# midas-journal/midas-journal-740

Measured on NVIDIA B200. Metric: Gvoxels/s, higher is better.
Workload: dtype f32

## Files before the change

### midas-journal-740_b200/csrc/cuberille_capi.cu

```cuda
#include <cuda_runtime.h>

#include <algorithm>
#include <cmath>
#include <cstdarg>
#include <cstdio>
#include <cstdlib>
#include <cstring>
#include <limits>
#include <new>
#include <string>
#include <type_traits>
#include <vector>

#include "../../include/cuberille_c.h"
#include "cbr_common.cuh"
#include "k_classify.cuh"
#include "k_segscan.cuh"
#include "k_generate.cuh"
#include "k_faces.cuh"
#include "k_project.cuh"
#include "k_sweep.cuh"
#include "k_fused.cuh"
#include "k_vertices.cuh"

// ... 827 lines not shown
  }
  const uint64_t tot_v = h->h_info[kInfoTotV], tot_f = h->h_info[kInfoTotF];
  if (tot_v >= (1ull << 32) || tot_f >= (1ull << 32))
    return fail(h, CUB_ERR_OVERFLOW, "more than 2^32 vertices or faces in one handle (%llu, %llu): split into z-slabs",
                (unsigned long long)tot_v, (unsigned long long)tot_f);
  h->n_active = h->h_info[kInfoTotC];
  h->ghost_f = h->h_info[kInfoMarkF];
  h->ghost_v = h->h_info[kInfoGhostV];
  h->n_points = h->h_info[kInfoPoints];
  h->n_quads = h->h_info[kInfoQuads];
  h->point_base = h->h_info[kInfoPointBase];
  h->cell_base = h->h_info[kInfoCellBase];
  h->flags = h->h_info[kInfoFlags];
  h->warning.clear();
  if (h->flags & kFlagEmptyInteriorSlice)
    h->warning = "an empty voxel slice lies between occupied slices: the reference filter merges vertices of different corner "
                 "planes there (its lookup-plane rotation only advances on inside voxels, txx:155-161); this mesh follows the "
                 "intended rule and may differ from the reference's";
  h->counted = true;
  return CUB_OK;
}

const int kNeedSizes = -1000;

int emit_mode(cub_handle h) {
  const cub_params& P = h->params;
  if (!P.generate_triangles) return kEmitQuads;
  return (P.project_vertices || h->geom.oriented) ? kEmitScratchQuads : kEmitTrisFixed;
}

int size_vertex_buffers(cub_handle h) {
  const size_t n_pts_all = (size_t)(h->ghost_v + h->n_points);
  CUB_TRY(ensure(h, h->points, 3 * (n_pts_all + n_pts_all / 16)));
  if (!h->raster) {
    CUB_TRY(ensure(h, h->perm, (size_t)h->n_active + (size_t)h->n_active / 16));
    CUB_TRY(ensure(h, h->vtx, h->points.cap / 3));
  }
  return CUB_OK;
}

int emit_vertex_stage(cub_handle h, bool exact) {
  const Grid& g = h->g;
  const int mode = emit_mode(h);
  const int nz = h->zs1 - h->owner_z_min;
  if (exact) {
    CUB_TRY(size_vertex_buffers(h));
    if (h->n_quads == 0) { h->vertices_done = true; return CUB_OK; }
  } else if (!h->points.p || (!h->raster && (!h->perm.p || !h->vtx.p))) {
    return kNeedSizes;
  }
  h->vertices_done = true;
  h->projected = false;
  if (!h->caps_checked) {
    CU_TRY(h, launch_step(h, k_check_caps, dim3(1), dim3(32), true, h->d_info, make_caps(h, ~0ull)));
  }
  const bool ghost_points = (mode == kEmitScratchQuads) && h->owner_z_min < h->zs0;
  if (!h->raster) {
    const size_t cap = std::min(h->points.cap / 3, h->vtx.cap);
    const size_t n_ids = exact ? (size_t)(h->ghost_v + h->n_points) : cap;
    const unsigned n_blocks = (unsigned)((n_ids + kVertexBlockIds - 1) / kVertexBlockIds);
    CUB_TRY(ensure(h, h->vsl, (size_t)nz + 1 + (cap + kVertexBlockIds - 1) / kVertexBlockIds + 1));
    {
      AssignArgs a{};
      a.cnt = h->cnt.p; a.own = h->own.p; a.seg = h->seg.p; a.cofs = h->cofs.p;
      a.Wx = g.Wx; a.EY = h->EY; a.EW = h->EW; a.NS = h->NS; a.z_begin = h->owner_z_min;
      a.ghost_row_end = (unsigned)((size_t)h->zs0 * h->EY);
      a.vtx = h->vtx.p; a.info = h->d_info;
      const int rows = kAssignThreads / 32;
      const dim3 grid((g.Wx + 31) / 32, (h->EY + rows - 1) / rows, nz + 1);
      CU_TRY(h, launch_step(h, k_assign, grid, dim3(kAssignThreads), true, a));
    }
    if (n_blocks > 0) {
      SliceIndexArgs si{};
      si.seg = h->seg.p; si.plane_segs = (size_t)h->EY * h->NS; si.z_first = h->owner_z_min; si.nz = nz;
      si.slice_first = h->vsl.p; si.block_slice = h->vsl.p + nz + 1; si.n_blocks = n_blocks; si.ids_per_block = kVertexBlockIds;
      const unsigned si_threads = n_blocks > (unsigned)nz + 1 ? n_blocks : (unsigned)nz + 1;
      CU_TRY(h, launch_step(h, k_slice_index, dim3((si_threads + 255) / 256), dim3(256), true, si));
      VertexArgs a{};
      a.vtx = h->vtx.p; a.caps = make_caps(h, ~0ull); a.write_ghost_points = ghost_points ? 1 : 0;
      a.info = h->d_info;
      a.slice_first = si.slice_first; a.block_slice = si.block_slice; a.z_first = h->owner_z_min;
      a.act = h->act.p; a.cofs = h->cofs.p; a.EY = h->EY; a.EW = h->EW;
      a.plane_lo = h->zs0; a.plane_hi = h->zs1; a.geom = h->geom;
      a.coff[0] = (int)(h->i0[0] - h->pad); a.coff[1] = (int)(h->i0[1] - h->pad); a.coff[2] = (int)(h->i0[2] + g.zg0 - h->pad);
      a.points = h->points.p; a.perm = h->perm.p;
      CU_TRY(h, launch_step(h, h->geom.oriented ? k_vertices<true> : k_vertices<false>, dim3(n_blocks), dim3(256), true, a));
    }
  } else {
    RasterPointArgs a{};
    a.act = h->act.p; a.cofs = h->cofs.p; a.seg = h->seg.p; a.EY = h->EY; a.EW = h->EW; a.NS = h->NS; a.Wc = (g.X + 32) / 32;
    a.plane_lo = h->zs0; a.plane_hi = h->zs1;
    a.point_plane_lo = (ghost_points || h->own_z0 == 0) ? h->zs0 : h->zs0 + 1;
    a.coff[0] = (int)(h->i0[0] - h->pad); a.coff[1] = (int)(h->i0[1] - h->pad); a.coff[2] = (int)(h->i0[2] + g.zg0 - h->pad);
    a.geom = h->geom; a.points = h->points.p; a.info = h->d_info;
    const dim3 grid((unsigned)h->NS, (h->EY + 7) / 8, a.plane_hi - a.plane_lo + 1);
    auto kern = h->geom.oriented ? k_points_raster<true> : k_points_raster<false>;
    kern<<<grid, 256, 0, h->stream>>>(a);
    h->launches++;
    CU_TRY(h, cudaGetLastError());
  }
  return CUB_OK;
}

int emit_launch(cub_handle h, int id_bytes, bool exact) {
  CU_TRY(h, cudaSetDevice(h->device));
  const cub_params& P = h->params;
  const Grid& g = h->g;
  const bool tri = P.generate_triangles != 0, proj = P.project_vertices != 0, cd = P.save_pixel_as_cell_data != 0;
  const int mode = emit_mode(h);
  h->verts_per_cell = tri ? 3 : 4;
  h->id_bytes = id_bytes;
  const size_t quad_bytes = (size_t)(tri ? 6 : 4) * id_bytes;
  const size_t cd_bytes = (size_t)(tri ? 2 : 1) * h->pix_bytes;
  if (exact) {
    h->n_cells = tri ? 2 * h->n_quads : h->n_quads;
    if (id_bytes == 4 && h->point_base + h->n_points > (1ull << 32))
      return fail(h, CUB_ERR_OVERFLOW, "point ids up to %llu do not fit 32 bits", (unsigned long long)(h->point_base + h->n_points));
    const size_t nq = (size_t)h->n_quads + (size_t)h->n_quads / 16;
    CUB_TRY(ensure(h, h->cells, nq * quad_bytes));
    if (mode == kEmitScratchQuads) CUB_TRY(ensure(h, h->quads, nq));
    if (cd) CUB_TRY(ensure(h, h->celldata, nq * cd_bytes));
  } else if (!h->cells.p || (mode == kEmitScratchQuads && !h->quads.p) || (cd && !h->celldata.p)) {
    return kNeedSizes;
  }
  size_t quads_cap = h->cells.cap / quad_bytes;
  if (mode == kEmitScratchQuads) quads_cap = std::min(quads_cap, h->quads.cap);
  if (cd) quads_cap = std::min(quads_cap, h->celldata.cap / cd_bytes);
  if (proj && h->projected) h->vertices_done = false;
  if (exact && !h->vertices_done) CUB_TRY(size_vertex_buffers(h));

  if (h->timing) cudaEventRecord(h->ev[4], h->stream);
  CU_TRY(h, launch_step(h, k_check_caps, dim3(1), dim3(32), true, h->d_info, make_caps(h, quads_cap)));
  h->caps_checked = true;
  const bool ghost_points = (mode == kEmitScratchQuads) && h->owner_z_min < h->zs0;
  if (!exact || h->n_quads > 0) {
    Timer t(h, 2);
    if (!h->vertices_done) {
      const int rc = emit_vertex_stage(h, exact);
      if (rc != CUB_OK) return rc;
    }
    {
      if (h->wait_before_faces) CU_TRY(h, cudaStreamWaitEvent(h->stream, h->wait_before_faces, 0));
      FaceArgs a{};
      a.bits = h->bits.p; a.g = g; a.EY = h->EY; a.EW = h->EW; a.NS = h->NS;
      a.z_begin = h->zs0; a.z_end = h->zs1;
      a.act = h->act.p; a.cofs = h->cofs.p; a.seg = h->seg.p; a.perm = h->raster ? nullptr : h->perm.p;
      a.info = h->d_info;
      a.cells = (mode == kEmitScratchQuads) ? (void*)h->quads.p : (void*)h->cells.p;
      a.mode = mode;
      a.vol = cd ? h->d_vol : nullptr;
      a.vX = h->gv.X; a.vY = h->gv.Y; a.vpad = h->pad; a.vzpad = h->zpad_lo;
      a.celldata = cd ? h->celldata.p : nullptr;
      a.pix_bytes = h->pix_bytes;
      const dim3 blocks((g.Wx + 31) / 32, (g.Y + kFaceThreads / 32 - 1) / (kFaceThreads / 32), h->zs1 - h->zs0);
      const bool pdl = h->wait_before_faces == nullptr;
      void (*kern)(FaceArgs);
      if (mode == kEmitScratchQuads) kern = cd ? k_faces<uint32_t, kEmitScratchQuads, true> : k_faces<uint32_t, kEmitScratchQuads, false>;
      else if (mode == kEmitQuads && id_bytes == 4) kern = cd ? k_faces<uint32_t, kEmitQuads, true> : k_faces<uint32_t, kEmitQuads, false>;
      else if (mode == kEmitQuads) kern = cd ? k_faces<unsigned long long, kEmitQuads, true> : k_faces<unsigned long long, kEmitQuads, false>;
      else if (id_bytes == 4) kern = cd ? k_faces<uint32_t, kEmitTrisFixed, true> : k_faces<uint32_t, kEmitTrisFixed, false>;
      else kern = cd ? k_faces<unsigned long long, kEmitTrisFixed, true> : k_faces<unsigned long long, kEmitTrisFixed, false>;
      CU_TRY(h, launch_step(h, kern, blocks, dim3(kFaceThreads), pdl, a));
    }
    t.stop();
  }
  if (proj && (!exact || h->n_points > 0)) {
    Timer t(h, 3);
    CUB_TRY(launch_project(h, h->points.p, h->points.cap / 3, true, ghost_points));
    h->projected = true;
    t.stop();
  }
  if (mode == kEmitScratchQuads && (!exact || h->n_quads > 0)) {
    Timer t(h, 4);
    const size_t want = exact ? (size_t)h->n_quads : quads_cap;
    const unsigned blocks = (unsigned)std::max<size_t>(1, std::min<size_t>((want + 255) / 256, (size_t)h->num_sms * 16));
    if (id_bytes == 4)
      k_split_quads<uint32_t><<<blocks, 256, 0, h->stream>>>(h->quads.p, h->points.p, (uint32_t*)h->cells.p, h->d_info);
    else
      k_split_quads<unsigned long long><<<blocks, 256, 0, h->stream>>>(h->quads.p, h->points.p, (unsigned long long*)h->cells.p, h->d_info);
    h->launches++;
    CU_TRY(h, cudaGetLastError());
    t.stop();
  }
  if (h->timing) {
    cudaEventRecord(h->ev[5], h->stream);
    cudaEventSynchronize(h->ev[5]);
    cudaEventElapsedTime(&h->ms[6], h->ev[4], h->ev[5]);
  }
  h->emitted = true;
  h->emit_unverified = !exact;
  return CUB_OK;
}

int verify_emit(cub_handle h) {
  if (!h->counted) CUB_TRY(count_finish(h));
  if (h->emit_unverified) {
    h->emit_unverified = false;
    const cub_params& P = h->params;
    h->n_cells = P.generate_triangles ? 2 * h->n_quads : h->n_quads;
    if (h->flags & kFlagBufferOverflow) {
      h->vertices_done = false;
      CUB_TRY(emit_launch(h, h->id_bytes, true));
      CU_TRY(h, cudaStreamSynchronize(h->stream));
    } else if (h->id_bytes == 4 && h->point_base + h->n_points > (1ull << 32)) {
      return fail(h, CUB_ERR_OVERFLOW, "point ids up to %llu do not fit 32 bits", (unsigned long long)(h->point_base + h->n_points));
    }
  }
  return CUB_OK;
}

}

extern "C" {

int cub_count(cub_handle h, const cub_params* p, uint64_t* n_points, uint64_t* n_quads) {
  if (!h) return CUB_ERR_INVALID;
  CUB_TRY(count_launch(h, p));
  CUB_TRY(count_finish(h));
  if (n_points) *n_points = h->n_points;
  if (n_quads) *n_quads = h->n_quads;
  return CUB_OK;
}

int cub_count_async(cub_handle h, const cub_params* p) {
  if (!h) return CUB_ERR_INVALID;
  return count_launch(h, p);
}

int cub_projection_halo(const cub_params* p, const double spacing[3], uint64_t* below, uint64_t* above) {
  if (!p || !below || !above) return CUB_ERR_INVALID;
  double sp[3] = {1.0, 1.0, 1.0};
  if (spacing) for (int a = 0; a < 3; ++a) sp[a] = spacing[a];
  if (!p->project_vertices) { *below = 2; *above = 1; return CUB_OK; }
  double ms = sp[0];
  for (int a = 1; a < 3; ++a) ms = sp[a] > ms ? sp[a] : ms;
  const double step = p->step_length < 0.0 ? ms * 0.25 : p->step_length;
  projection_reach(*p, step, 1.0 / sp[2], below, above);
  return CUB_OK;
}

int cub_set_id_base(cub_handle h, uint64_t point_id_base, uint64_t cell_id_base) {
  if (!h) return CUB_ERR_INVALID;
  h->point_base = point_id_base;
  h->cell_base = cell_id_base;
  if (h->count_queued) {
    CU_TRY(h, cudaSetDevice(h->device));
    k_set_bases<<<1, 32, 0, h->stream>>>(h->d_info, point_id_base, cell_id_base);
    h->launches++;
    CU_TRY(h, cudaGetLastError());
  }
  return CUB_OK;
}

int cub_emit_vertices(cub_handle h) {
  if (!h) return CUB_ERR_INVALID;
  if (!h->count_queued) return fail(h, CUB_ERR_INVALID, "cub_emit_vertices before cub_count");
  CU_TRY(h, cudaSetDevice(h->device));
  if (h->vertices_done || h->timing) return CUB_OK;
  const int rc = emit_vertex_stage(h, h->counted);
  return rc == kNeedSizes ? CUB_OK : rc;
}

int cub_emit(cub_handle h, int id_bytes) {
  if (!h) return CUB_ERR_INVALID;
  if (!h->count_queued) return fail(h, CUB_ERR_INVALID, "cub_emit before cub_count");
  if (id_bytes != 4 && id_bytes != 8) return fail(h, CUB_ERR_INVALID, "id_bytes must be 4 or 8");
  if (!h->counted) CUB_TRY(count_finish(h));
  return emit_launch(h, id_bytes, true);
}

int cub_emit_async(cub_handle h, int id_bytes) {
  if (!h) return CUB_ERR_INVALID;
  if (!h->count_queued) return fail(h, CUB_ERR_INVALID, "cub_emit_async before cub_count_async");
  if (id_bytes != 4 && id_bytes != 8) return fail(h, CUB_ERR_INVALID, "id_bytes must be 4 or 8");
  if (!h->counted && !h->timing) {
    const int rc = emit_launch(h, id_bytes, false);
    if (rc != kNeedSizes) return rc;
  }
  if (!h->counted) CUB_TRY(count_finish(h));
  return emit_launch(h, id_bytes, true);
}

int cub_finish(cub_handle h, uint64_t* n_points, uint64_t* n_cells) {
  if (!h) return CUB_ERR_INVALID;
  if (!h->count_queued) return fail(h, CUB_ERR_INVALID, "cub_finish: nothing has been queued");
  CUB_TRY(verify_emit(h));
  if (!h->emit_unverified) CU_TRY(h, cudaStreamSynchronize(h->stream));
  if (n_points) *n_points = h->n_points;
  if (n_cells) *n_cells = h->params.generate_triangles ? 2 * h->n_quads : h->n_quads;
  return CUB_OK;
}

int cub_device_counts(cub_handle h, const uint64_t** counts) {
  if (!h || !counts) return CUB_ERR_INVALID;
  *counts = reinterpret_cast<const uint64_t*>(h->d_info + kInfoPoints);
  return CUB_OK;
}

const char* cub_last_warning(cub_handle h) { return h ? h->warning.c_str() : ""; }

int cub_run(cub_handle h, const cub_params* p, int id_bytes, uint64_t* n_points, uint64_t* n_cells) {
  uint64_t np = 0, nq = 0;
  CUB_TRY(cub_count(h, p, &np, &nq));
  CUB_TRY(cub_emit(h, id_bytes));
  if (n_points) *n_points = h->n_points;
  if (n_cells) *n_cells = h->n_cells;
  return CUB_OK;
// ... 201 lines not shown
```

### midas-journal-740_b200/csrc/k_faces.cuh

```cuda
#pragma once
#include "cbr_common.cuh"
#include "k_segscan.cuh"

namespace cbr {

enum { kEmitQuads = 0, kEmitTrisFixed = 1, kEmitScratchQuads = 2 };

struct FaceArgs {
  const uint32_t* bits;
  Grid g;
  int EY, EW, NS;
  int z_begin, z_end;
  const uint32_t* act;
  const uint32_t* cofs;
  const uint4* seg;
  const uint32_t* perm;
  unsigned long long* info;
  void* cells;
  int mode;
  const void* vol;
  int vX, vY, vpad, vzpad;
  void* celldata;
  int pix_bytes;
};

template <typename IdT>
__device__ __forceinline__ void store_tri_pair(IdT* c, IdT a0, IdT a1, IdT a2, IdT b0, IdT b1, IdT b2) {
  if (sizeof(IdT) == 4) {
    uint2* d = reinterpret_cast<uint2*>(c);
    d[0] = make_uint2((uint32_t)a0, (uint32_t)a1);
    d[1] = make_uint2((uint32_t)a2, (uint32_t)b0);
    d[2] = make_uint2((uint32_t)b1, (uint32_t)b2);
  } else {
    ulonglong2* d = reinterpret_cast<ulonglong2*>(c);
    d[0] = make_ulonglong2((unsigned long long)a0, (unsigned long long)a1);
    d[1] = make_ulonglong2((unsigned long long)a2, (unsigned long long)b0);
    d[2] = make_ulonglong2((unsigned long long)b1, (unsigned long long)b2);
  }
}

template <typename IdT, int MODE>
__device__ __forceinline__ void write_cell(const FaceArgs& a, uint32_t fidx, IdT v0, IdT v1, IdT v2, IdT v3) {
  if (MODE == kEmitScratchQuads) {
    reinterpret_cast<uint4*>(a.cells)[fidx] = make_uint4((uint32_t)v0, (uint32_t)v1, (uint32_t)v2, (uint32_t)v3);
    return;
  }
  IdT* c = reinterpret_cast<IdT*>(a.cells);
  if (MODE == kEmitQuads) {
    c += (size_t)fidx * 4;
    if (sizeof(IdT) == 4) {
      *reinterpret_cast<uint4*>(c) = make_uint4((uint32_t)v0, (uint32_t)v1, (uint32_t)v2, (uint32_t)v3);
    } else {
      reinterpret_cast<ulonglong2*>(c)[0] = make_ulonglong2((unsigned long long)v0, (unsigned long long)v1);
      reinterpret_cast<ulonglong2*>(c)[1] = make_ulonglong2((unsigned long long)v2, (unsigned long long)v3);
    }
  } else {
    c += (size_t)fidx * 6;
    store_tri_pair<IdT>(c, v0, v1, v3, v1, v2, v3);
  }
}

__device__ __forceinline__ unsigned long long load_pixel(const void* vol, size_t voxel, int pix_bytes) {
  switch (pix_bytes) {
    case 1: return __ldg(reinterpret_cast<const uint8_t*>(vol) + voxel);
    case 2: return __ldg(reinterpret_cast<const uint16_t*>(vol) + voxel);
    case 4: return __ldg(reinterpret_cast<const uint32_t*>(vol) + voxel);
    default: return __ldg(reinterpret_cast<const unsigned long long*>(vol) + voxel);
  }
}

template <int MODE>
__device__ __forceinline__ void write_celldata(const FaceArgs& a, uint32_t fidx, unsigned long long pix) {
  const bool two = (MODE != kEmitQuads);
  const size_t c = two ? 2 * (size_t)fidx : (size_t)fidx;
  switch (a.pix_bytes) {
    case 1: { uint8_t* d = reinterpret_cast<uint8_t*>(a.celldata) + c; d[0] = (uint8_t)pix; if (two) d[1] = (uint8_t)pix; break; }
    case 2: { uint16_t* d = reinterpret_cast<uint16_t*>(a.celldata) + c; d[0] = (uint16_t)pix; if (two) d[1] = (uint16_t)pix; break; }
    case 4: { uint32_t* d = reinterpret_cast<uint32_t*>(a.celldata) + c; d[0] = (uint32_t)pix; if (two) d[1] = (uint32_t)pix; break; }
    default: { unsigned long long* d = reinterpret_cast<unsigned long long*>(a.celldata) + c; d[0] = pix; if (two) d[1] = pix; break; }
  }
}

constexpr int kFaceThreads = 128;

struct FaceSmem {
  uint4 ctx[4][kFaceThreads / 32][32];
  uint16_t queue[kFaceThreads / 32][1024];
};

template <typename IdT, int MODE, bool CD>
__global__ void __launch_bounds__(kFaceThreads, 12) k_faces(const FaceArgs a) {
  pdl_enter();
  __shared__ FaceSmem sm;
  const bool fits = emission_fits(a.info);
  const Grid& g = a.g;
  const int lane = threadIdx.x & 31, warp = threadIdx.x >> 5;
  const int sgm = blockIdx.x, w = sgm * 32 + lane, y = blockIdx.y * (kFaceThreads / 32) + warp, zl = a.z_begin + blockIdx.z;

  uint32_t F[6] = {0, 0, 0, 0, 0, 0};
  const int plane = a.EY * a.EW;
  const uint32_t e00 = ((uint32_t)zl * (uint32_t)a.EY + (uint32_t)y) * (uint32_t)a.EW + (uint32_t)w;
  uint32_t A[4] = {0, 0, 0, 0}, C[4] = {0, 0, 0, 0};
  uint32_t fseg = 0;
  const unsigned long long id_delta = __ldg(a.info + kInfoIdDelta);
  const uint32_t ghost_f = (uint32_t)__ldg(a.info + kInfoMarkF);
  {
    const bool valid = w < g.Wx && y < g.Y;
    if (y < g.Y) fseg = __ldg(&a.seg[((uint32_t)zl * (uint32_t)a.EY + (uint32_t)y) * (uint32_t)a.NS + (uint32_t)sgm].y);
    const uint32_t* __restrict__ row = a.bits + (((uint32_t)zl * (uint32_t)g.Y + (uint32_t)y) * (uint32_t)g.Wp + (uint32_t)w);
    const int zgl = zl + g.zg0;
    const int sw = g.Y * g.Wp;
    const int dym = (y > 0) ? -g.Wp : 0, dyp = (y < g.Y - 1) ? g.Wp : 0;
    const int dzm = (zgl > 0 && zl > 0) ? -sw : 0, dzp = (zgl < g.Zg - 1 && zl < g.Zl - 1) ? sw : 0;
    uint32_t c0 = 0, nym = 0, nyp = 0, nzm = 0, nzp = 0, edge = 0;
    if (valid) {
#pragma unroll
      for (int k = 0; k < 4; ++k) {
        const uint32_t e = e00 + (uint32_t)((k >> 1) * plane + (k & 1) * a.EW);
        A[k] = __ldg(a.act + e);
        C[k] = __ldg(a.cofs + e);
      }
      c0 = __ldg(row);
      nym = __ldg(row + dym); nyp = __ldg(row + dyp); nzm = __ldg(row + dzm); nzp = __ldg(row + dzp);
      if (lane == 0 && w > 0) edge = __ldg(row - 1);
      if (lane == 31 && w < g.Wx - 1) edge = __ldg(row + 1);
    }
    const uint32_t up = __shfl_up_sync(0xffffffffu, c0, 1), dn = __shfl_down_sync(0xffffffffu, c0, 1);
    if (valid) {
      const uint32_t XB = g.X & 31;
      const uint32_t vc = (w == g.Wx - 1 && XB) ? ((1u << XB) - 1u) : ~0u;
      const uint32_t c = c0 & vc;
      const uint32_t prev = (w == 0) ? (c0 << 31) : (lane == 0 ? edge : up);
      const uint32_t next = (w == g.Wx - 1) ? (c0 >> 31) : (lane == 31 ? edge : dn);
      F[0] = c & ~__funnelshift_l(prev, c0, 1);
      F[1] = c & ~nym;
      F[2] = c & ~__funnelshift_r(c0, next, 1);
      F[3] = c & ~nyp;
      F[4] = c & ~nzm;
      F[5] = c & ~nzp;
    }
  }
  uint32_t U = F[0] | F[1] | F[2] | F[3] | F[4] | F[5];
  const uint32_t nvox = __popc(U);
  const uint32_t nf = __popc(F[0]) + __popc(F[1]) + __popc(F[2]) + __popc(F[3]) + __popc(F[4]) + __popc(F[5]);
  uint32_t s0 = nvox | (nf << 16);
  const uint32_t m0 = s0;
#pragma unroll
  for (int o = 1; o < 32; o <<= 1) {
    const uint32_t t0 = __shfl_up_sync(0xffffffffu, s0, o);
    if (lane >= o) s0 += t0;
  }
  const uint32_t total = __shfl_sync(0xffffffffu, s0, 31) & 0xffffu;
  if (!fits) return;
  if (total == 0) return;

  if (U) {
    s0 -= m0;
    sm.ctx[0][warp][lane] = make_uint4(A[0], A[1], A[2], A[3]);
    sm.ctx[1][warp][lane] = make_uint4(C[0], C[1], C[2], C[3]);
    sm.ctx[2][warp][lane] = make_uint4(F[0], F[1], F[2], F[3]);
    sm.ctx[3][warp][lane] = make_uint4(F[4], F[5], fseg + (s0 >> 16) - ghost_f, 0u);
    uint32_t pos = s0 & 0xffffu;
    uint16_t* q = sm.queue[warp];
    const uint32_t tag = (uint32_t)lane << 5;
    while (U) {
      const int b = __ffs(U) - 1;
      U &= U - 1;
      q[pos++] = (uint16_t)(tag | (uint32_t)b);
    }
  }
  __syncwarp();

  for (uint32_t s = lane; s < total; s += 32) {
    const uint32_t it = sm.queue[warp][s];
    const uint32_t src = it >> 5, b = it & 31u;
    const uint4 A4 = sm.ctx[0][warp][src], C4 = sm.ctx[1][warp][src], Fa = sm.ctx[2][warp][src], Fb = sm.ctx[3][warp][src];
    const uint32_t A[4] = {A4.x, A4.y, A4.z, A4.w}, C[4] = {C4.x, C4.y, C4.z, C4.w};
    const uint32_t Fm[6] = {Fa.x, Fa.y, Fa.z, Fa.w, Fb.x, Fb.y};
    const uint32_t bit = 1u << b, below = bit - 1u;
    uint32_t fi = Fb.z;
#pragma unroll
    for (int f = 0; f < 6; ++f) fi += __popc(Fm[f] & below);
    uint32_t vid[8];
#pragma unroll
    for (int k = 0; k < 4; ++k) {
      const int oz = k >> 1, oy = k & 1;
      const uint32_t s0 = C[k] + __popc(A[k] & below);
      const uint32_t s1 = s0 + ((A[k] >> b) & 1u);
      vid[oz * 4 + (oy ? 3 : 0)] = s0;
      vid[oz * 4 + (oy ? 2 : 1)] = s1;
    }
    const bool f0 = Fm[0] & bit, f1 = Fm[1] & bit, f2 = Fm[2] & bit, f3 = Fm[3] & bit, f4 = Fm[4] & bit, f5 = Fm[5] & bit;
    if (a.perm) {
      const bool need[8] = {f0 || f1 || f4, f1 || f2 || f4, f2 || f3 || f4, f0 || f3 || f4,
                            f0 || f1 || f5, f1 || f2 || f5, f2 || f3 || f5, f0 || f3 || f5};
#pragma unroll
      for (int l = 0; l < 8; ++l)
        if (need[l]) vid[l] = __ldg(a.perm + vid[l]);
    }
    const unsigned long long voxel =
        CD ? load_pixel(a.vol, ((size_t)(zl - a.vzpad) * a.vY + (size_t)(y - a.vpad)) * a.vX +
                                           (size_t)((sgm * 32 + src) * 32 + b - a.vpad), a.pix_bytes) : 0ull;
    IdT fid[8];
#pragma unroll
    for (int l = 0; l < 8; ++l) fid[l] = MODE == kEmitScratchQuads ? (IdT)vid[l] : (IdT)(vid[l] + id_delta);
    if (f0) { write_cell<IdT, MODE>(a, fi, fid[0], fid[4], fid[7], fid[3]); if (CD) write_celldata<MODE>(a, fi, voxel); ++fi; }
    if (f1) { write_cell<IdT, MODE>(a, fi, fid[0], fid[1], fid[5], fid[4]); if (CD) write_celldata<MODE>(a, fi, voxel); ++fi; }
    if (f2) { write_cell<IdT, MODE>(a, fi, fid[1], fid[2], fid[6], fid[5]); if (CD) write_celldata<MODE>(a, fi, voxel); ++fi; }
    if (f3) { write_cell<IdT, MODE>(a, fi, fid[2], fid[3], fid[7], fid[6]); if (CD) write_celldata<MODE>(a, fi, voxel); ++fi; }
    if (f4) { write_cell<IdT, MODE>(a, fi, fid[0], fid[3], fid[2], fid[1]); if (CD) write_celldata<MODE>(a, fi, voxel); ++fi; }
    if (f5) { write_cell<IdT, MODE>(a, fi, fid[4], fid[5], fid[6], fid[7]); if (CD) write_celldata<MODE>(a, fi, voxel); ++fi; }
  }
}

template <typename IdT>
__global__ void __launch_bounds__(256) k_split_quads(const uint4* __restrict__ quads, const float* __restrict__ points,
                                                     IdT* __restrict__ tris, unsigned long long* __restrict__ info) {
  if (!emission_fits(info)) return;
  const size_t n_quads = (size_t)__ldg(info + kInfoQuads);
  const unsigned long long id_delta = __ldg(info + kInfoIdDelta);
  for (size_t i = (size_t)blockIdx.x * blockDim.x + threadIdx.x; i < n_quads; i += (size_t)gridDim.x * blockDim.x) {
    const uint4 q = quads[i];
    const uint32_t id[4] = {q.x, q.y, q.z, q.w};
    float p[4][3];
#pragma unroll
    for (int k = 0; k < 4; ++k)
#pragma unroll
      for (int c = 0; c < 3; ++c) p[k][c] = __ldg(points + 3 * (size_t)id[k] + c);
    double d02 = 0.0, d13 = 0.0;
#pragma unroll
    for (int c = 0; c < 3; ++c) {
      const double a = __dadd_rn((double)p[0][c], -(double)p[2][c]);
      d02 = __dadd_rn(d02, __dmul_rn(a, a));
      const double b = __dadd_rn((double)p[1][c], -(double)p[3][c]);
      d13 = __dadd_rn(d13, __dmul_rn(b, b));
    }
    IdT v[4];
#pragma unroll
    for (int k = 0; k < 4; ++k) v[k] = (IdT)((unsigned long long)id[k] + id_delta);
    IdT* c = tris + i * 6;
    const bool first = d02 >= d13;
    store_tri_pair<IdT>(c, v[0], v[1], first ? v[3] : v[2], first ? v[1] : v[0], v[2], v[3]);
  }
}

}
```

Baseline: 540.8.

## Process four bit-words per lane in face kernel with chunked queue and batched emission

Each lane of the face-emission kernel now handles four consecutive 32-bit occupancy words, loaded with uint4 vector loads, so a warp covers four rows instead of one. The per-warp voxel queue becomes a 512-entry ring that is filled and drained in chunks. Emission gathers two queued voxels before writing, so the perm and pixel loads can overlap. The goal is fewer load instructions, more work per thread and better latency hiding, at the cost of higher register and shared-memory use, which is why occupancy is lowered from 12 to 5 blocks per SM.

```diff
diff --git a/midas-journal-740_b200/csrc/cuberille_capi.cu b/midas-journal-740_b200/csrc/cuberille_capi.cu
--- a/midas-journal-740_b200/csrc/cuberille_capi.cu
+++ b/midas-journal-740_b200/csrc/cuberille_capi.cu
@@ -1003,7 +1003,7 @@
       a.vX = h->gv.X; a.vY = h->gv.Y; a.vpad = h->pad; a.vzpad = h->zpad_lo;
       a.celldata = cd ? h->celldata.p : nullptr;
       a.pix_bytes = h->pix_bytes;
-      const dim3 blocks((g.Wx + 31) / 32, (g.Y + kFaceThreads / 32 - 1) / (kFaceThreads / 32), h->zs1 - h->zs0);
+      const dim3 blocks((g.Wx + 31) / 32, (g.Y + kFaceRows - 1) / kFaceRows, h->zs1 - h->zs0);
       const bool pdl = h->wait_before_faces == nullptr;
       void (*kern)(FaceArgs);
       if (mode == kEmitScratchQuads) kern = cd ? k_faces<uint32_t, kEmitScratchQuads, true> : k_faces<uint32_t, kEmitScratchQuads, false>;
diff --git a/midas-journal-740_b200/csrc/k_faces.cuh b/midas-journal-740_b200/csrc/k_faces.cuh
--- a/midas-journal-740_b200/csrc/k_faces.cuh
+++ b/midas-journal-740_b200/csrc/k_faces.cuh
@@ -82,67 +82,167 @@
 }
 
 constexpr int kFaceThreads = 128;
+constexpr int kFaceWordsPerLane = 4;
+constexpr int kFaceLanesPerSeg = 32 / kFaceWordsPerLane;
+constexpr int kFaceSegsPerWarp = 32 / kFaceLanesPerSeg;
+constexpr int kFaceRows = kFaceThreads / 32 * kFaceSegsPerWarp;
+constexpr int kFaceSlots = 32 * kFaceWordsPerLane;
+constexpr int kFaceQueue = 512;
+constexpr int kFaceEmitDepth = 2;
 
 struct FaceSmem {
-  uint4 ctx[4][kFaceThreads / 32][32];
-  uint16_t queue[kFaceThreads / 32][1024];
+  uint4 ctx[4][kFaceThreads / 32][kFaceSlots];
+  uint16_t queue[kFaceThreads / 32][kFaceQueue];
 };
 
+__device__ __forceinline__ uint32_t u4_get(const uint4& v, int j) {
+  return j == 0 ? v.x : (j == 1 ? v.y : (j == 2 ? v.z : v.w));
+}
+
+struct QueuedVoxel {
+  uint32_t fi, faces;
+  uint32_t vid[8];
+  unsigned long long pix;
+};
+
+template <bool CD>
+__device__ __forceinline__ QueuedVoxel gather_voxel(const FaceArgs& a, const FaceSmem& sm, int warp, uint32_t it, bool valid,
+                                                    int sgm, int y0, int zl) {
+  QueuedVoxel v;
+  const uint32_t src = it >> 5, b = it & 31u;
+  const uint4 A4 = sm.ctx[0][warp][src], C4 = sm.ctx[1][warp][src], Fa = sm.ctx[2][warp][src], Fb = sm.ctx[3][warp][src];
+  const uint32_t A[4] = {A4.x, A4.y, A4.z, A4.w}, C[4] = {C4.x, C4.y, C4.z, C4.w};
+  const uint32_t Fm[6] = {Fa.x, Fa.y, Fa.z, Fa.w, Fb.x, Fb.y};
+  const uint32_t bit = 1u << b, below = bit - 1u;
+  v.fi = Fb.z;
+  v.faces = 0;
+#pragma unroll
+  for (int f = 0; f < 6; ++f) {
+    v.fi += __popc(Fm[f] & below);
+    v.faces |= ((Fm[f] >> b) & 1u) << f;
+  }
+  if (!valid) v.faces = 0;
+#pragma unroll
+  for (int k = 0; k < 4; ++k) {
+    const int oz = k >> 1, oy = k & 1;
+    const uint32_t s0 = C[k] + __popc(A[k] & below);
+    const uint32_t s1 = s0 + ((A[k] >> b) & 1u);
+    v.vid[oz * 4 + (oy ? 3 : 0)] = s0;
+    v.vid[oz * 4 + (oy ? 2 : 1)] = s1;
+  }
+  const bool f0 = v.faces & 1u, f1 = v.faces & 2u, f2 = v.faces & 4u, f3 = v.faces & 8u, f4 = v.faces & 16u, f5 = v.faces & 32u;
+  if (a.perm) {
+    const bool need[8] = {f0 || f1 || f4, f1 || f2 || f4, f2 || f3 || f4, f0 || f3 || f4,
+                          f0 || f1 || f5, f1 || f2 || f5, f2 || f3 || f5, f0 || f3 || f5};
+#pragma unroll
+    for (int l = 0; l < 8; ++l)
+      if (need[l]) v.vid[l] = __ldg(a.perm + v.vid[l]);
+  }
+  v.pix = 0;
+  if (CD && valid) {
+    const int sl = (int)(src & 31u), sj = (int)(src >> 5);
+    const int y = y0 + sl / kFaceLanesPerSeg, w = sgm * 32 + (sl % kFaceLanesPerSeg) * kFaceWordsPerLane + sj;
+    v.pix = load_pixel(a.vol, ((size_t)(zl - a.vzpad) * a.vY + (size_t)(y - a.vpad)) * a.vX +
+                                  (size_t)(w * 32 + (int)b - a.vpad), a.pix_bytes);
+  }
+  return v;
+}
+
 template <typename IdT, int MODE, bool CD>
-__global__ void __launch_bounds__(kFaceThreads, 12) k_faces(const FaceArgs a) {
+__device__ __forceinline__ void write_voxel(const FaceArgs& a, const QueuedVoxel& v, unsigned long long id_delta) {
+  IdT fid[8];
+#pragma unroll
+  for (int l = 0; l < 8; ++l) fid[l] = MODE == kEmitScratchQuads ? (IdT)v.vid[l] : (IdT)(v.vid[l] + id_delta);
+  uint32_t fi = v.fi;
+  if (v.faces & 1u) { write_cell<IdT, MODE>(a, fi, fid[0], fid[4], fid[7], fid[3]); if (CD) write_celldata<MODE>(a, fi, v.pix); ++fi; }
+  if (v.faces & 2u) { write_cell<IdT, MODE>(a, fi, fid[0], fid[1], fid[5], fid[4]); if (CD) write_celldata<MODE>(a, fi, v.pix); ++fi; }
+  if (v.faces & 4u) { write_cell<IdT, MODE>(a, fi, fid[1], fid[2], fid[6], fid[5]); if (CD) write_celldata<MODE>(a, fi, v.pix); ++fi; }
+  if (v.faces & 8u) { write_cell<IdT, MODE>(a, fi, fid[2], fid[3], fid[7], fid[6]); if (CD) write_celldata<MODE>(a, fi, v.pix); ++fi; }
+  if (v.faces & 16u) { write_cell<IdT, MODE>(a, fi, fid[0], fid[3], fid[2], fid[1]); if (CD) write_celldata<MODE>(a, fi, v.pix); ++fi; }
+  if (v.faces & 32u) { write_cell<IdT, MODE>(a, fi, fid[4], fid[5], fid[6], fid[7]); if (CD) write_celldata<MODE>(a, fi, v.pix); ++fi; }
+}
+
+template <typename IdT, int MODE, bool CD>
+__global__ void __launch_bounds__(kFaceThreads, 5) k_faces(const FaceArgs a) {
   pdl_enter();
   __shared__ FaceSmem sm;
   const bool fits = emission_fits(a.info);
   const Grid& g = a.g;
   const int lane = threadIdx.x & 31, warp = threadIdx.x >> 5;
-  const int sgm = blockIdx.x, w = sgm * 32 + lane, y = blockIdx.y * (kFaceThreads / 32) + warp, zl = a.z_begin + blockIdx.z;
-
-  uint32_t F[6] = {0, 0, 0, 0, 0, 0};
-  const int plane = a.EY * a.EW;
-  const uint32_t e00 = ((uint32_t)zl * (uint32_t)a.EY + (uint32_t)y) * (uint32_t)a.EW + (uint32_t)w;
-  uint32_t A[4] = {0, 0, 0, 0}, C[4] = {0, 0, 0, 0};
+  const int sub = lane % kFaceLanesPerSeg;
+  const int sgm = blockIdx.x, w0 = sgm * 32 + sub * kFaceWordsPerLane;
+  const int y = blockIdx.y * kFaceRows + warp * kFaceSegsPerWarp + lane / kFaceLanesPerSeg, zl = a.z_begin + blockIdx.z;
+
+  uint32_t F[kFaceWordsPerLane][6];
+  uint4 A[4], C[4];
   uint32_t fseg = 0;
   const unsigned long long id_delta = __ldg(a.info + kInfoIdDelta);
   const uint32_t ghost_f = (uint32_t)__ldg(a.info + kInfoMarkF);
   {
-    const bool valid = w < g.Wx && y < g.Y;
+    const bool live = w0 < g.Wx && y < g.Y;
     if (y < g.Y) fseg = __ldg(&a.seg[((uint32_t)zl * (uint32_t)a.EY + (uint32_t)y) * (uint32_t)a.NS + (uint32_t)sgm].y);
-    const uint32_t* __restrict__ row = a.bits + (((uint32_t)zl * (uint32_t)g.Y + (uint32_t)y) * (uint32_t)g.Wp + (uint32_t)w);
+    const uint32_t* __restrict__ row = a.bits + (((uint32_t)zl * (uint32_t)g.Y + (uint32_t)y) * (uint32_t)g.Wp + (uint32_t)w0);
+    const int plane = a.EY * a.EW;
+    const uint32_t e00 = ((uint32_t)zl * (uint32_t)a.EY + (uint32_t)y) * (uint32_t)a.EW + (uint32_t)w0;
     const int zgl = zl + g.zg0;
     const int sw = g.Y * g.Wp;
     const int dym = (y > 0) ? -g.Wp : 0, dyp = (y < g.Y - 1) ? g.Wp : 0;
     const int dzm = (zgl > 0 && zl > 0) ? -sw : 0, dzp = (zgl < g.Zg - 1 && zl < g.Zl - 1) ? sw : 0;
-    uint32_t c0 = 0, nym = 0, nyp = 0, nzm = 0, nzp = 0, edge = 0;
-    if (valid) {
+    const uint4 z4 = make_uint4(0u, 0u, 0u, 0u);
+    uint4 c4 = z4, nym = z4, nyp = z4, nzm = z4, nzp = z4;
+    uint32_t edge = 0;
+#pragma unroll
+    for (int k = 0; k < 4; ++k) A[k] = C[k] = z4;
+    if (live) {
 #pragma unroll
       for (int k = 0; k < 4; ++k) {
         const uint32_t e = e00 + (uint32_t)((k >> 1) * plane + (k & 1) * a.EW);
-        A[k] = __ldg(a.act + e);
-        C[k] = __ldg(a.cofs + e);
+        A[k] = __ldg(reinterpret_cast<const uint4*>(a.act + e));
+        C[k] = __ldg(reinterpret_cast<const uint4*>(a.cofs + e));
       }
-      c0 = __ldg(row);
-      nym = __ldg(row + dym); nyp = __ldg(row + dyp); nzm = __ldg(row + dzm); nzp = __ldg(row + dzp);
-      if (lane == 0 && w > 0) edge = __ldg(row - 1);
-      if (lane == 31 && w < g.Wx - 1) edge = __ldg(row + 1);
-    }
-    const uint32_t up = __shfl_up_sync(0xffffffffu, c0, 1), dn = __shfl_down_sync(0xffffffffu, c0, 1);
-    if (valid) {
-      const uint32_t XB = g.X & 31;
-      const uint32_t vc = (w == g.Wx - 1 && XB) ? ((1u << XB) - 1u) : ~0u;
-      const uint32_t c = c0 & vc;
-      const uint32_t prev = (w == 0) ? (c0 << 31) : (lane == 0 ? edge : up);
-      const uint32_t next = (w == g.Wx - 1) ? (c0 >> 31) : (lane == 31 ? edge : dn);
-      F[0] = c & ~__funnelshift_l(prev, c0, 1);
-      F[1] = c & ~nym;
-      F[2] = c & ~__funnelshift_r(c0, next, 1);
-      F[3] = c & ~nyp;
-      F[4] = c & ~nzm;
-      F[5] = c & ~nzp;
-    }
-  }
-  uint32_t U = F[0] | F[1] | F[2] | F[3] | F[4] | F[5];
-  const uint32_t nvox = __popc(U);
-  const uint32_t nf = __popc(F[0]) + __popc(F[1]) + __popc(F[2]) + __popc(F[3]) + __popc(F[4]) + __popc(F[5]);
+      c4 = __ldg(reinterpret_cast<const uint4*>(row));
+      nym = __ldg(reinterpret_cast<const uint4*>(row + dym)); nyp = __ldg(reinterpret_cast<const uint4*>(row + dyp));
+      nzm = __ldg(reinterpret_cast<const uint4*>(row + dzm)); nzp = __ldg(reinterpret_cast<const uint4*>(row + dzp));
+      if (sub == 0 && w0 > 0) edge = __ldg(row - 1);
+      if (sub == kFaceLanesPerSeg - 1 && w0 + kFaceWordsPerLane < g.Wx) edge = __ldg(row + kFaceWordsPerLane);
+    }
+    const uint32_t up = __shfl_up_sync(0xffffffffu, c4.w, 1), dn = __shfl_down_sync(0xffffffffu, c4.x, 1);
+    const uint32_t XB = g.X & 31;
+#pragma unroll
+    for (int j = 0; j < kFaceWordsPerLane; ++j) {
+      const int w = w0 + j;
+      const uint32_t c0 = u4_get(c4, j);
+#pragma unroll
+      for (int f = 0; f < 6; ++f) F[j][f] = 0;
+      if (live && w < g.Wx) {
+        const uint32_t vc = (w == g.Wx - 1 && XB) ? ((1u << XB) - 1u) : ~0u;
+        const uint32_t c = c0 & vc;
+        const uint32_t prev = j > 0 ? u4_get(c4, j - 1) : ((w == 0) ? (c0 << 31) : (sub == 0 ? edge : up));
+        const uint32_t next = (w == g.Wx - 1) ? (c0 >> 31)
+                                              : (j < kFaceWordsPerLane - 1 ? u4_get(c4, j + 1)
+                                                                           : (sub == kFaceLanesPerSeg - 1 ? edge : dn));
+        F[j][0] = c & ~__funnelshift_l(prev, c0, 1);
+        F[j][1] = c & ~u4_get(nym, j);
+        F[j][2] = c & ~__funnelshift_r(c0, next, 1);
+        F[j][3] = c & ~u4_get(nyp, j);
+        F[j][4] = c & ~u4_get(nzm, j);
+        F[j][5] = c & ~u4_get(nzp, j);
+      }
+    }
+  }
+  uint32_t U[kFaceWordsPerLane], nfw[kFaceWordsPerLane];
+  uint32_t nvox = 0, nf = 0;
+#pragma unroll
+  for (int j = 0; j < kFaceWordsPerLane; ++j) {
+    U[j] = F[j][0] | F[j][1] | F[j][2] | F[j][3] | F[j][4] | F[j][5];
+    nfw[j] = __popc(F[j][0]) + __popc(F[j][1]) + __popc(F[j][2]) + __popc(F[j][3]) + __popc(F[j][4]) + __popc(F[j][5]);
+    nvox += __popc(U[j]);
+    nf += nfw[j];
+    const int slot = j * 32 + lane;
+    sm.ctx[0][warp][slot] = make_uint4(u4_get(A[0], j), u4_get(A[1], j), u4_get(A[2], j), u4_get(A[3], j));
+    sm.ctx[1][warp][slot] = make_uint4(u4_get(C[0], j), u4_get(C[1], j), u4_get(C[2], j), u4_get(C[3], j));
+    sm.ctx[2][warp][slot] = make_uint4(F[j][0], F[j][1], F[j][2], F[j][3]);
+  }
   uint32_t s0 = nvox | (nf << 16);
   const uint32_t m0 = s0;
 #pragma unroll
@@ -154,62 +254,41 @@
   if (!fits) return;
   if (total == 0) return;
 
-  if (U) {
-    s0 -= m0;
-    sm.ctx[0][warp][lane] = make_uint4(A[0], A[1], A[2], A[3]);
-    sm.ctx[1][warp][lane] = make_uint4(C[0], C[1], C[2], C[3]);
-    sm.ctx[2][warp][lane] = make_uint4(F[0], F[1], F[2], F[3]);
-    sm.ctx[3][warp][lane] = make_uint4(F[4], F[5], fseg + (s0 >> 16) - ghost_f, 0u);
-    uint32_t pos = s0 & 0xffffu;
-    uint16_t* q = sm.queue[warp];
-    const uint32_t tag = (uint32_t)lane << 5;
-    while (U) {
-      const int b = __ffs(U) - 1;
-      U &= U - 1;
-      q[pos++] = (uint16_t)(tag | (uint32_t)b);
-    }
-  }
-  __syncwarp();
-
-  for (uint32_t s = lane; s < total; s += 32) {
-    const uint32_t it = sm.queue[warp][s];
-    const uint32_t src = it >> 5, b = it & 31u;
-    const uint4 A4 = sm.ctx[0][warp][src], C4 = sm.ctx[1][warp][src], Fa = sm.ctx[2][warp][src], Fb = sm.ctx[3][warp][src];
-    const uint32_t A[4] = {A4.x, A4.y, A4.z, A4.w}, C[4] = {C4.x, C4.y, C4.z, C4.w};
-    const uint32_t Fm[6] = {Fa.x, Fa.y, Fa.z, Fa.w, Fb.x, Fb.y};
-    const uint32_t bit = 1u << b, below = bit - 1u;
-    uint32_t fi = Fb.z;
-#pragma unroll
-    for (int f = 0; f < 6; ++f) fi += __popc(Fm[f] & below);
-    uint32_t vid[8];
-#pragma unroll
-    for (int k = 0; k < 4; ++k) {
-      const int oz = k >> 1, oy = k & 1;
-      const uint32_t s0 = C[k] + __popc(A[k] & below);
-      const uint32_t s1 = s0 + ((A[k] >> b) & 1u);
-      vid[oz * 4 + (oy ? 3 : 0)] = s0;
-      vid[oz * 4 + (oy ? 2 : 1)] = s1;
-    }
-    const bool f0 = Fm[0] & bit, f1 = Fm[1] & bit, f2 = Fm[2] & bit, f3 = Fm[3] & bit, f4 = Fm[4] & bit, f5 = Fm[5] & bit;
-    if (a.perm) {
-      const bool need[8] = {f0 || f1 || f4, f1 || f2 || f4, f2 || f3 || f4, f0 || f3 || f4,
-                            f0 || f1 || f5, f1 || f2 || f5, f2 || f3 || f5, f0 || f3 || f5};
-#pragma unroll
-      for (int l = 0; l < 8; ++l)
-        if (need[l]) vid[l] = __ldg(a.perm + vid[l]);
-    }
-    const unsigned long long voxel =
-        CD ? load_pixel(a.vol, ((size_t)(zl - a.vzpad) * a.vY + (size_t)(y - a.vpad)) * a.vX +
-                                           (size_t)((sgm * 32 + src) * 32 + b - a.vpad), a.pix_bytes) : 0ull;
-    IdT fid[8];
-#pragma unroll
-    for (int l = 0; l < 8; ++l) fid[l] = MODE == kEmitScratchQuads ? (IdT)vid[l] : (IdT)(vid[l] + id_delta);
-    if (f0) { write_cell<IdT, MODE>(a, fi, fid[0], fid[4], fid[7], fid[3]); if (CD) write_celldata<MODE>(a, fi, voxel); ++fi; }
-    if (f1) { write_cell<IdT, MODE>(a, fi, fid[0], fid[1], fid[5], fid[4]); if (CD) write_celldata<MODE>(a, fi, voxel); ++fi; }
-    if (f2) { write_cell<IdT, MODE>(a, fi, fid[1], fid[2], fid[6], fid[5]); if (CD) write_celldata<MODE>(a, fi, voxel); ++fi; }
-    if (f3) { write_cell<IdT, MODE>(a, fi, fid[2], fid[3], fid[7], fid[6]); if (CD) write_celldata<MODE>(a, fi, voxel); ++fi; }
-    if (f4) { write_cell<IdT, MODE>(a, fi, fid[0], fid[3], fid[2], fid[1]); if (CD) write_celldata<MODE>(a, fi, voxel); ++fi; }
-    if (f5) { write_cell<IdT, MODE>(a, fi, fid[4], fid[5], fid[6], fid[7]); if (CD) write_celldata<MODE>(a, fi, voxel); ++fi; }
+  s0 -= m0;
+  const uint32_t seg_f0 = __shfl_sync(0xffffffffu, s0, lane & ~(kFaceLanesPerSeg - 1)) >> 16;
+  uint32_t fb = fseg + ((s0 >> 16) - seg_f0) - ghost_f;
+#pragma unroll
+  for (int j = 0; j < kFaceWordsPerLane; ++j) {
+    if (U[j]) sm.ctx[3][warp][j * 32 + lane] = make_uint4(F[j][4], F[j][5], fb, 0u);
+    fb += nfw[j];
+  }
+
+  uint16_t* q = sm.queue[warp];
+  uint32_t pos = s0 & 0xffffu;
+  for (uint32_t r0 = 0; r0 < total; r0 += kFaceQueue) {
+    const uint32_t r1 = min(total, r0 + (uint32_t)kFaceQueue);
+#pragma unroll
+    for (int j = 0; j < kFaceWordsPerLane; ++j) {
+      const uint32_t tag = (uint32_t)(j * 32 + lane) << 5;
+      while (U[j] && pos < r1) {
+        const int b = __ffs(U[j]) - 1;
+        U[j] &= U[j] - 1;
+        q[pos++ - r0] = (uint16_t)(tag | (uint32_t)b);
+      }
+    }
+    __syncwarp();
+    for (uint32_t s = r0 + lane; s < r1; s += 32 * kFaceEmitDepth) {
+      QueuedVoxel v[kFaceEmitDepth];
+#pragma unroll
+      for (int u = 0; u < kFaceEmitDepth; ++u) {
+        const uint32_t su = s + 32u * u;
+        const bool valid = su < r1;
+        v[u] = gather_voxel<CD>(a, sm, warp, q[valid ? su - r0 : 0], valid, sgm, y - lane / kFaceLanesPerSeg, zl);
+      }
+#pragma unroll
+      for (int u = 0; u < kFaceEmitDepth; ++u) write_voxel<IdT, MODE, CD>(a, v[u], id_delta);
+    }
+    __syncwarp();
   }
 }
 
```

Result: slower. 533.8 (median of 6 runs) (-1.3%).
